# TheoBald200814/RGB-D-Instance-Segmentation

Measured on AMD Instinct MI355X. Metric: NYUv2 640x480 RGB-D img/s (fwd+bwd) of the DGGM+E-DSAM hot path, higher is better.
Workload: dtype bf16

## Files before the change

### rgb-d-instance-segmentation_amd/csrc/ratio_common.hpp

```cpp
#pragma once
#include <algorithm>

#include "mfma.hpp"
#include "timing.hpp"

namespace rgbd::rp {

constexpr int STEM_K = 160, STEM_C = 192, FUS_C = 128, ATT_C = 64, C5 = 256, C6 = 512;
constexpr int STEM_K2 = 168;
constexpr int NBN = 6;
constexpr float BN_EPS = 1e-5f;

struct Layout {
  size_t w1, b1, w2, b2, w3, b3, w4, b4, w5, b5, w6, b6, w7, b7, w8, b8, w9, b9, w10, b10;
  size_t zero;
  size_t w5q;
  size_t w1s;
  size_t w1f, w2f;
  size_t total;
};

inline Layout make_layout(int es) {
  Layout L;
  size_t o = 0;
  auto seg = [&](size_t bytes) {
    size_t r = o;
    o += align256(bytes);
    return r;
  };
  L.w1 = seg((size_t)STEM_C * STEM_K * es);
  L.b1 = seg(STEM_C * 4);
  L.w2 = seg((size_t)FUS_C * STEM_C * es);
  L.b2 = seg(FUS_C * 4);
  L.w3 = seg((size_t)ATT_C * FUS_C * es);
  L.b3 = seg(ATT_C * 4);
  L.w4 = seg((size_t)FUS_C * ATT_C * es);
  L.b4 = seg(FUS_C * 4);
  L.w5 = seg((size_t)C5 * 9 * FUS_C * es);
  L.b5 = seg(C5 * 4);
  L.w6 = seg((size_t)C6 * C5 * 9 * 4);
  L.b6 = seg(C6 * 4);
  L.w7 = seg(128 * 512 * 4);
  L.b7 = seg(128 * 4);
  L.w8 = seg(64 * 128 * 4);
  L.b8 = seg(64 * 4);
  L.w9 = seg(32 * 64 * 4);
  L.b9 = seg(32 * 4);
  L.w10 = seg(32 * 4);
  L.b10 = seg(4);
  L.zero = seg(256);
  L.w1s = seg(es == 2 ? (size_t)STEM_C * STEM_K2 * 2 : 0);
  L.w1f = seg(es == 2 ? (size_t)STEM_C * STEM_K2 * 4 : 0);
  L.w2f = seg(es == 2 ? (size_t)FUS_C * STEM_C * 4 : 0);
  L.w5q = seg(es == 2 ? (size_t)C5 * 9 * FUS_C * 2 : 0);
  L.total = o;
  return L;
}

__host__ __device__ __forceinline__ int chain_perm(int g, int e) { return e < 4 ? 4 * g + e : 16 + 4 * g + (e - 4); }

struct WPtrs {
  const float* p[RGBD_RATIO_NW];
};
struct BnPtrs {
  float* p[NBN * 4];
};

constexpr int CH_TW = 16, CH_TH = 4;
constexpr int C2W_TH = 8, C2W_TW = 32, C2W_PH = C2W_TH + 6, C2W_PW = C2W_TW + 6;
constexpr int C2W_S1 = STEM_K2 + 8, C2W_S2 = STEM_C + 8, C2W_S3 = FUS_C + 8, C2W_S4 = ATT_C + 8;
constexpr int CV_TH = 4, CV_TW = 32;
constexpr int C4_TH = 16, C4_TW = 32, C4_PW = C4_TW + 2;
constexpr int POOL_SPLIT = 16;
constexpr size_t FOLD_W1 = 0, FOLD_W2 = FOLD_W1 + (size_t)STEM_C * STEM_K2 * 2;
constexpr size_t FOLD_B1 = FOLD_W2 + (size_t)FUS_C * STEM_C * 2, FOLD_B2 = FOLD_B1 + STEM_C * 4;
constexpr size_t FOLD_BYTES = FOLD_B2 + FUS_C * 4;
inline bool stem_moments_ok(int H, int W) { return H >= 8 && W >= 8; }

__host__ __device__ __forceinline__ int c4_ph(int H) { return (H + 15) / 16 * 16 + 2; }
__host__ __device__ __forceinline__ int c4_pw(int W) { return (W + 31) / 32 * 32 + 2; }
__host__ __device__ __forceinline__ long long c4_att_idx(int b, int q, int y, int x, int H, int W) {
  return (((long long)b * 4 + q) * c4_ph(H) + y + 1) * c4_pw(W) * 32 + (long long)(x + 1) * 32;
}

struct TileDec {
  int b, y0, x0;
};
__device__ __forceinline__ TileDec tile_dec(unsigned t, unsigned per, unsigned tiles_x, int th, int tw) {
  const unsigned b = t / per, rem = t - b * per, ty = rem / tiles_x;
  return TileDec{(int)b, (int)ty * th, (int)(rem - ty * tiles_x) * tw};
}

__device__ __forceinline__ float sigmoid_fast(float x) {
  return __builtin_amdgcn_rcpf(1.f + __builtin_amdgcn_exp2f(-1.4426950408889634f * x));
}

struct BnVals {
  float g, b, rm, rv;
};
__device__ __forceinline__ BnVals bn_vals(const float* gamma, const float* beta, const float* run_mean,
                                          const float* run_var, int c) {
  return BnVals{gamma[c], beta[c], run_mean[c], run_var[c]};
}
__device__ __forceinline__ float2 bn_finish_v(double s, double q, double count, int training, float momentum,
                                              const BnVals& p, float* run_mean, float* run_var, int c,
                                              float2* __restrict__ affine) {
  float mean, var;
  if (training) {
    const double m = s / count;
    double v = q / count - m * m;
    if (v < 0.0) v = 0.0;
    mean = (float)m;
    var = (float)v;
    const double unb = count > 1.0 ? v * count / (count - 1.0) : v;
    run_mean[c] = (1.f - momentum) * p.rm + momentum * mean;
    run_var[c] = (1.f - momentum) * p.rv + momentum * (float)unb;
  } else {
    mean = p.rm;
    var = p.rv;
  }
  const float sc = p.g / sqrtf(var + BN_EPS);
  const float2 af = make_float2(sc, p.b - mean * sc);
  affine[c] = af;
  return af;
}
__device__ __forceinline__ float2 bn_finish(double s, double q, double count, int training, float momentum,
                                            const float* gamma, const float* beta, float* run_mean, float* run_var,
                                            int c, float2* __restrict__ affine) {
  return bn_finish_v(s, q, count, training, momentum, bn_vals(gamma, beta, run_mean, run_var, c), run_mean, run_var,
                     c, affine);
}
__device__ __forceinline__ void bn_affine_body(const float* __restrict__ slab, int nslab, int row, int c_off, int c,
                                               double count, int training, float momentum, const float* gamma,
                                               const float* beta, float* run_mean, float* run_var,
                                               float2* __restrict__ affine, int cm = 0) {
  __shared__ double red[2][4];
  BnVals pv{};
  if (threadIdx.x == 0) pv = bn_vals(gamma, beta, run_mean, run_var, c);
  double s = 0.0, q = 0.0;
  if (training) {
    int i = threadIdx.x;
    for (; i + 256 * 7 < nslab; i += 256 * 8) {
      float2 v[8];
#pragma unroll
      for (int u = 0; u < 8; ++u)
        v[u] = *reinterpret_cast<const float2*>(
            slab + (cm ? (long long)(c_off + c) * nslab + i + 256 * u : (long long)(i + 256 * u) * row + c_off + c) * 2);
#pragma unroll
      for (int u = 0; u < 8; ++u) {
        s += (double)v[u].x;
        q += (double)v[u].y;
      }
    }
    for (; i < nslab; i += 256) {
      const long long e = cm ? (long long)(c_off + c) * nslab + i : (long long)i * row + c_off + c;
      s += (double)slab[e * 2 + 0];
      q += (double)slab[e * 2 + 1];
    }
  }
  s = wave_sum_f64(s);
  q = wave_sum_f64(q);
  if ((threadIdx.x & 63) == 0) {
    red[0][threadIdx.x >> 6] = s;
    red[1][threadIdx.x >> 6] = q;
  }
  __syncthreads();
  if (threadIdx.x != 0) return;
  bn_finish_v(((red[0][0] + red[0][1]) + red[0][2]) + red[0][3], ((red[1][0] + red[1][1]) + red[1][2]) + red[1][3],
              count, training, momentum, pv, run_mean, run_var, c, affine);
}

__device__ inline void c4_pad_body(bf16_t* __restrict__ att, int H, int W, int bx, int plane, int nbx) {
  const int PH = c4_ph(H), PW = c4_pw(W);
  bf16_t* pl = att + (long long)plane * PH * PW * 32;
  const int edge_rows = PH - H, side = PW - W;
  const long long full = (long long)edge_rows * PW * 4, part = (long long)H * side * 4;
  for (long long i = bx * 256 + threadIdx.x; i < full + part; i += 256LL * nbx) {
    long long px;
    if (i < full) {
      const long long c = i >> 2;
      const int rr = (int)(c / PW), cc = (int)(c % PW);
      px = (long long)(rr == 0 ? 0 : H + rr) * PW + cc;
    } else {
      const long long c = (i - full) >> 2;
      const int rr = (int)(c / side), k = (int)(c % side);
      px = (long long)(rr + 1) * PW + (k == 0 ? 0 : W + k);
    }
    *reinterpret_cast<uint4*>(pl + px * 32 + 8 * (i & 3)) = make_uint4(0u, 0u, 0u, 0u);
  }
}

inline int device_cus() {
  static int n = [] {
    int dev = 0, v = 0;
    if (hipGetDevice(&dev) != hipSuccess || hipDeviceGetAttribute(&v, hipDeviceAttributeMultiprocessorCount, dev) != hipSuccess)
      v = 256;
    return v > 0 ? v : 256;
  }();
  return n;
}


int bn_affine(const float* slab, int nslab, int C, double count, int training, float momentum, const BnPtrs& bn,
              int layer, float2* affine, int cm, hipStream_t s);
int bn_affine_stem(const float* slab, int nslab, double count, int training, float momentum, const BnPtrs& bn,
                   float2* aff1, hipStream_t s);
size_t stem_ws_size(int B, int H, int W);
int stem_bn_moments(const float* depth3, long long bstride, int B, int H, int W, const char* blob, const Layout& L,
                    float momentum, const BnPtrs& bn, float2* aff1, char* fold, bf16_t* att, char* ws, hipStream_t s);

int chain_grid_v2(int B, int H, int W, int phase = 1);
int fold_bn(const char* blob, const Layout& L, const float2* aff, int which, char* fold, hipStream_t s);
int chain_v2(int phase, const float* depth3, long long bstride, int B, int H, int W, const char* blob, const Layout& L,
             const float2* aff1, const float2* aff2, const char* fold, float* slab, bf16_t* att, hipStream_t s);

int gate(const bf16_t* fus, int B, int H, int W, const char* blob, const Layout& L, const float2* aff2, bf16_t* att,
         hipStream_t s);
int c4_pad_zero(bf16_t* att, int B, int H, int W, hipStream_t s);
long long conv4_tiles(int B, int H, int W);
int conv4_grid(int B, int H, int W);
bool conv4_pool_fused(int H, int W);
int conv5_v4(int mode, const bf16_t* att, int B, int H, int W, const char* blob, const Layout& L, const float2* aff5,
             bf16_t* y, float* out, hipStream_t s);
int pool_v4(const bf16_t* y, int B, int H, int W, const float2* aff5, float* part, hipStream_t s);
int pool_finish_v4(const float* ip, int B, int H, int W, float* pooled, hipStream_t s);

int chain_grid(int B, int H, int W);
int conv_grid(int B, int H, int W);
int chain_f32(int phase, const float* depth3, long long bstride, int B, int H, int W, const char* blob,
              const Layout& L, const float2* aff1, const float2* aff2, float* slab, float* att, hipStream_t s);
int conv3x3_f32(const float* att, int B, int H, int W, const char* blob, const Layout& L, float* y, float* slab,
                hipStream_t s);
int bn_relu_pool_f32(const float* y, int B, int H, int W, const float2* aff5, float* part, hipStream_t s);

int pool_finish(const float* part, int B, int H, int W, float* pooled, hipStream_t s);
int tail(const float* pooled, int B, int training, float momentum, const char* blob, const Layout& L,
         const BnPtrs& bn, unsigned long long seed, unsigned long long* seed_ctr, float* feat, float* h1, float* ratio,
         hipStream_t s);

}
```

### rgb-d-instance-segmentation_amd/csrc/ratio_conv5.hip

```cpp
#include "ratio_common.hpp"

using namespace rgbd;
using namespace rgbd::rp;

namespace {

constexpr int GT_S = FUS_C + 8;
constexpr size_t GT_OFF_W3 = 0;
constexpr size_t GT_OFF_W4 = GT_OFF_W3 + (size_t)ATT_C * C2W_S3 * 2;
constexpr size_t GT_OFF_B = GT_OFF_W4 + (size_t)FUS_C * C2W_S4 * 2;
constexpr size_t GT_OFF_IMG = GT_OFF_B + (size_t)(ATT_C + FUS_C + 2 * FUS_C) * 4;
constexpr size_t GT_SMEM = GT_OFF_IMG + (size_t)8 * C2W_TW * GT_S * 2;
static_assert(GT_SMEM <= 163840, "gate LDS budget");

__global__ __launch_bounds__(512) void k_rp_gate(const bf16_t* __restrict__ fus, int B, int H, int W,
                                                 const char* __restrict__ blob, Layout L,
                                                 const float2* __restrict__ aff2, bf16_t* __restrict__ att) {
  extern __shared__ __attribute__((aligned(16))) char smem[];
  const bf16_t* sW3 = (const bf16_t*)(smem + GT_OFF_W3);
  const bf16_t* sW4 = (const bf16_t*)(smem + GT_OFF_W4);
  float* sb3 = (float*)(smem + GT_OFF_B);
  float* sb4 = sb3 + ATT_C;
  float2* saff = (float2*)(sb4 + FUS_C);
  const int tid = threadIdx.x, lane = tid & 63, wave = tid >> 6;
  const int r = lane & 15, g = lane >> 4;
  bf16_t* img = (bf16_t*)(smem + GT_OFF_IMG) + (size_t)wave * C2W_TW * GT_S;
  {
    auto copy_rows = [&](size_t dst, size_t src, int rows, int k, int stride) {
      const int per = k / 8;
      for (int i = tid; i < rows * per; i += 512) {
        const int rr = i / per, q = i % per;
        *reinterpret_cast<uint4*>(smem + dst + ((size_t)rr * stride + 8 * q) * 2) =
            *reinterpret_cast<const uint4*>(blob + src + ((size_t)rr * k + 8 * q) * 2);
      }
    };
    copy_rows(GT_OFF_W3, L.w3, ATT_C, FUS_C, C2W_S3);
    copy_rows(GT_OFF_W4, L.w4, FUS_C, ATT_C, C2W_S4);
    for (int i = tid; i < ATT_C; i += 512) sb3[i] = ((const float*)(blob + L.b3))[i];
    for (int i = tid; i < FUS_C; i += 512) {
      sb4[i] = ((const float*)(blob + L.b4))[i];
      saff[i] = aff2[i];
    }
  }
  __syncthreads();
  const int tiles_x = (W + C2W_TW - 1) / C2W_TW, tiles_y = (H + C2W_TH - 1) / C2W_TH;
  const unsigned per = (unsigned)(tiles_x * tiles_y);
  const int ntiles = B * tiles_x * tiles_y;
  uint2 nxt[8][2];
  auto fetch = [&](int tl) {
    if (tl >= ntiles) return;
    const int tp = ntiles - 1 - tl;
    const bf16_t* ft = fus + (((long long)tp * 8 + wave) * 16) * 256;
#pragma unroll
    for (int t = 0; t < 8; ++t) {
      const u32x4 q = __builtin_nontemporal_load(reinterpret_cast<const u32x4*>(ft + (t * 64 + lane) * 8));
      nxt[t][0] = make_uint2(q[0], q[1]);
      nxt[t][1] = make_uint2(q[2], q[3]);
    }
  };
  fetch(blockIdx.x);
  for (int tile = blockIdx.x; tile < ntiles; tile += gridDim.x) {
    const TileDec td = tile_dec((unsigned)(ntiles - 1 - tile), per, (unsigned)tiles_x, C2W_TH, C2W_TW);
    const int b = td.b, y0 = td.y0, x0 = td.x0;
    const int py = y0 + wave;
    uint2 raw[8][2];
#pragma unroll
    for (int t = 0; t < 8; ++t)
#pragma unroll
      for (int u = 0; u < 2; ++u) raw[t][u] = nxt[t][u];
    fetch(tile + gridDim.x);
    if (py >= H) continue;
    asm volatile("s_waitcnt lgkmcnt(0)" ::: "memory");
#pragma unroll
    for (int t = 0; t < 8; ++t) {
      const int c = 16 * t + r;
      const float2 a = saff[c];
#pragma unroll
      for (int u = 0; u < 2; ++u) {
        const uint32_t w01 = raw[t][u].x, w23 = raw[t][u].y;
        const float v[4] = {__uint_as_float(w01 << 16), __uint_as_float(w01 & 0xffff0000u),
                            __uint_as_float(w23 << 16), __uint_as_float(w23 & 0xffff0000u)};
#pragma unroll
        for (int j = 0; j < 4; ++j)
          img[(16 * u + 4 * g + j) * GT_S + c] = f32_to_bf16(fmaxf(__builtin_fmaf(v[j], a.x, a.y), 0.f));
      }
    }
    __builtin_amdgcn_wave_barrier();
    asm volatile("s_waitcnt lgkmcnt(0)" ::: "memory");
    Frag<bf16_t> f2[4][2];
#pragma unroll
    for (int s = 0; s < 4; ++s)
#pragma unroll
      for (int u = 0; u < 2; ++u) {
        const bf16_t* row = img + (16 * u + r) * GT_S + 32 * s + 4 * g;
        const uint2 lo = *reinterpret_cast<const uint2*>(row), hi = *reinterpret_cast<const uint2*>(row + 16);
        f2[s][u].v = make_uint4(lo.x, lo.y, hi.x, hi.y);
      }
    f32x4 a3[4][2];
#pragma unroll
    for (int t = 0; t < 4; ++t) {
      const float4 bb = *reinterpret_cast<const float4*>(sb3 + 16 * t + 4 * g);
      a3[t][0] = a3[t][1] = f32x4{bb.x, bb.y, bb.z, bb.w};
#pragma unroll
      for (int s = 0; s < 4; ++s) {
        Frag<bf16_t> af;
        af.v = *reinterpret_cast<const uint4*>(sW3 + (16 * t + r) * C2W_S3 + 32 * s + 8 * g);
        mma(a3[t][0], af, f2[s][0]);
        mma(a3[t][1], af, f2[s][1]);
      }
    }
    Frag<bf16_t> f3[2][2];
#pragma unroll
    for (int s = 0; s < 2; ++s)
#pragma unroll
      for (int u = 0; u < 2; ++u) {
        float vv[8];
#pragma unroll
        for (int e = 0; e < 8; ++e) vv[e] = fmaxf(a3[2 * s + (e >> 2)][u][e & 3], 0.f);
        f3[s][u].from8(vv);
      }
#pragma unroll
    for (int t = 0; t < 8; ++t) {
      const float4 bb = *reinterpret_cast<const float4*>(sb4 + 16 * t + 4 * g);
      f32x4 a4[2] = {f32x4{bb.x, bb.y, bb.z, bb.w}, f32x4{bb.x, bb.y, bb.z, bb.w}};
#pragma unroll
      for (int s = 0; s < 2; ++s) {
        Frag<bf16_t> af;
        af.v = *reinterpret_cast<const uint4*>(sW4 + (16 * t + r) * C2W_S4 + 32 * s + 8 * g);
        mma(a4[0], af, f3[s][0]);
        mma(a4[1], af, f3[s][1]);
      }
#pragma unroll
      for (int u = 0; u < 2; ++u) {
        uint2* cell = reinterpret_cast<uint2*>(img + (16 * u + r) * GT_S + 16 * t + 4 * g);
        const uint2 act = *cell;
        const float av[4] = {__uint_as_float(act.x << 16), __uint_as_float(act.x & 0xffff0000u),
                             __uint_as_float(act.y << 16), __uint_as_float(act.y & 0xffff0000u)};
        float o[4];
#pragma unroll
        for (int j = 0; j < 4; ++j) o[j] = av[j] * sigmoid_fast(a4[u][j]);
        *cell = make_uint2(pack_bf16x2(o[0], o[1]), pack_bf16x2(o[2], o[3]));
      }
    }
    __builtin_amdgcn_wave_barrier();
    asm volatile("s_waitcnt lgkmcnt(0)" ::: "memory");
#pragma unroll
    for (int k = 0; k < 8; ++k) {
      const int qt = k >> 1, pr = 16 * (k & 1) + (lane >> 2), q = lane & 3;
      if (x0 + pr < W)
        *reinterpret_cast<uint4*>(att + c4_att_idx(b, qt, py, x0 + pr, H, W) + 8 * q) =
            *reinterpret_cast<const uint4*>(img + pr * GT_S + 32 * qt + 8 * q);
    }
  }
}

constexpr int C4_NPIX = (C4_TH + 2) * C4_PW;
constexpr int C4_APIECES = 39;
constexpr int C4_A_BYTES = C4_APIECES * 1024;
constexpr int C4_STEPS = 12;
constexpr int C4_B_BYTES = 3 * 128 * 64;
constexpr int C4_B_OFF = 2 * C4_A_BYTES;
constexpr int C4_RED_OFF = C4_B_OFF + 2 * C4_B_BYTES;
constexpr int C4_RED_BYTES = 8 * 4 * 128 * 4;
constexpr int C4_PAR_OFF = C4_RED_OFF + C4_RED_BYTES;
constexpr size_t C4_SMEM = C4_PAR_OFF + 128 * 4 + 128 * 8 + 32 * 4;
static_assert(C4_SMEM <= 163840, "conv5 v4 LDS budget");
static_assert(C4_APIECES * 16 >= C4_NPIX && C4_APIECES % 3 == 0, "conv5 v4 input pieces");
constexpr int C4_AK = (C4_APIECES + 3) / 4;
static_assert(2 * C4_A_BYTES >= 8 * 128 * 2 * 4, "conv5 v4 statistics scratch");

__device__ __forceinline__ uint32_t c4_off(int row, int chunk) { return row * 64 + 16 * (chunk ^ ((row >> 1) & 2)); }

struct C4Tile {
  int b, y0, x0;
};
__device__ __forceinline__ C4Tile c4_tile(long long t, int tiles_x, int tiles_y) {
  C4Tile o;
  const long long per = (long long)tiles_x * tiles_y;
  o.b = (int)(t / per);
  const int rem = (int)(t % per);
  o.y0 = (rem / tiles_x) * C4_TH;
  o.x0 = (rem % tiles_x) * C4_TW;
  return o;
}

#ifndef C4_NODMA
#define C4_NODMA 0
#endif


#if defined(RGBD_DIAG) && !defined(C4_STAMPS)
#define C4_STAMPS
#endif
#ifdef C4_STAMPS
__device__ unsigned long long* g_c4_stamps = nullptr;
__device__ __forceinline__ void c4_stamp(unsigned long long* st, long long idx) {
  __builtin_amdgcn_sched_barrier(0);
  const unsigned long long t = __builtin_amdgcn_s_memtime();
  if ((threadIdx.x & 63) == 0) st[idx] = t;
  __builtin_amdgcn_sched_barrier(0);
}
#define C4_STAMP(k) \
  if (sts) c4_stamp(sts, (((long long)tcount * C4_STEPS + st) * 8 + wave) * 5 + (k))
#else
#define C4_STAMP(k)
#endif
template <int MODE>
__global__ __launch_bounds__(512) void k_rp_conv5_v4(const bf16_t* __restrict__ x, int B, int H, int W,
                                                     const char* __restrict__ blob, Layout L,
                                                     const float2* __restrict__ aff, bf16_t* __restrict__ y,
                                                     float* __restrict__ out, int xcd_pairs) {
  extern __shared__ __attribute__((aligned(1024))) char smem[];
  const int tid = threadIdx.x, lane = tid & 63;
  const int wave = __builtin_amdgcn_readfirstlane(tid >> 6);
  const int r = lane & 15, g = lane >> 4;
  const uint32_t lds0 = (uint32_t)(uintptr_t)smem;
  int pair, nh;
  if (xcd_pairs) {
    nh = (blockIdx.x >> 3) & 1;
    pair = (blockIdx.x & 7) | ((blockIdx.x >> 4) << 3);
  } else {
    nh = blockIdx.x & 1;
    pair = blockIdx.x >> 1;
  }
  const int npairs = gridDim.x >> 1;
  const char* w5q = blob + L.w5q + (size_t)nh * C4_STEPS * C4_B_BYTES;
  float* sbias = (float*)(smem + C4_PAR_OFF);
  float2* saff = (float2*)(smem + C4_PAR_OFF + 512);
  int* sslot = (int*)(smem + C4_PAR_OFF + 512 + 1024);
  for (int i = tid; i < 128; i += 512) {
    sbias[i] = ((const float*)(blob + L.b5))[nh * 128 + i];
    if constexpr (MODE == 1) saff[i] = aff[nh * 128 + i];
  }
  const int tiles_x = (W + C4_TW - 1) / C4_TW, tiles_y = (H + C4_TH - 1) / C4_TH;
  const long long ntiles = (long long)B * tiles_x * tiles_y;

  const int PW = c4_pw(W);
  const long long plane = (long long)c4_ph(H) * PW * 32;
  uint32_t aoff[C4_AK];
#pragma unroll
  for (int k = 0; k < C4_AK; ++k) {
    const int row = 16 * ((wave & 3) + 4 * k) + (lane >> 2), q = lane & 3;
    const int hy = row / C4_PW, hx = row - hy * C4_PW;
    aoff[k] = row < C4_NPIX ? (uint32_t)((hy * PW + hx) * 64 + 16 * (q ^ ((row >> 1) & 2))) : 0u;
  }
  auto issue_a = [&](const C4Tile& t, int qt, int sl, int k) {
    const char* base = (const char*)(x + ((long long)t.b * 4 + qt) * plane + ((long long)t.y0 * PW + t.x0) * 32);
    dma_lds16(base + aoff[k], lds0 + sl * C4_A_BYTES + ((wave & 3) + 4 * k) * 1024);
  };
  auto issue_b = [&](int st, int k0, int k1) {
    const char* src = w5q + (size_t)st * C4_B_BYTES + 16 * lane;
    const uint32_t dst = lds0 + C4_B_OFF + (st & 1) * C4_B_BYTES;
    for (int k = k0; k < k1; ++k) dma_lds16(src + 1024 * k, dst + 1024 * k);
  };
  const bool loader = wave < 4;

  f32x2 ssum[8], ssq[8];
#pragma unroll
  for (int nj = 0; nj < 8; ++nj) ssum[nj] = ssq[nj] = f32x2{0.f, 0.f};
  const int rh = H >> 2, rw = W >> 2;

#ifndef C4_NOPRIO
  if (wave >= 4) __builtin_amdgcn_s_setprio(1);
#endif
  long long tile = pair;
  if (tile < ntiles) {
    const C4Tile t = c4_tile(tile, tiles_x, tiles_y);
    if (!loader) {
#pragma unroll
      for (int k = 0; k < C4_AK; ++k)
        if ((wave & 3) + 4 * k < C4_APIECES) issue_a(t, 0, 0, k);
    }
    issue_b(0, 3 * wave, 3 * wave + 3);
  }
  asm volatile("s_waitcnt vmcnt(0)" ::: "memory");
  __syncthreads();

#ifdef C4_STAMPS
  int tcount = 0;
#endif
  for (; tile < ntiles; tile += npairs) {
#ifdef C4_STAMPS
    unsigned long long* const sts = (blockIdx.x == 0 && tcount < 2) ? g_c4_stamps : nullptr;
#endif
    const C4Tile t = c4_tile(tile, tiles_x, tiles_y);
    const long long ntile = tile + npairs;
    const bool has_next = ntile < ntiles;
    const C4Tile tn = c4_tile(has_next ? ntile : tile, tiles_x, tiles_y);
    f32x4 acc[4][8];
#pragma unroll
    for (int mi = 0; mi < 4; ++mi)
#pragma unroll
      for (int nj = 0; nj < 8; ++nj) acc[mi][nj] = f32x4{0.f, 0.f, 0.f, 0.f};

#pragma unroll 1
    for (int st = 0; st < C4_STEPS; ++st) {
      const int qt = st / 3, ky = st - 3 * qt;
      C4_STAMP(0);
      if (!(C4_NODMA & 1) && loader && (st + 1 < C4_STEPS || has_next))
        issue_b(st + 1 < C4_STEPS ? st + 1 : 0, 6 * wave, 6 * wave + 6);
      C4_STAMP(1);
      const int qn = qt + 1;
      const bool a_go = !(C4_NODMA & 2) && !loader && (qn < 4 || has_next);
      const char* sa = smem + (qt & 1) * C4_A_BYTES;
      const char* sb = smem + C4_B_OFF + (st & 1) * C4_B_BYTES;
#pragma unroll
      for (int kx = 0; kx < 3; ++kx) {
        Frag<bf16_t> fa[4], fb[8];
        if constexpr (!(C4_NODMA & 8)) {
#pragma unroll
          for (int mi = 0; mi < 4; ++mi) {
            const int p = (2 * wave + (mi >> 1) + ky) * C4_PW + (mi & 1) * 16 + r + kx;
            fa[mi].v = *reinterpret_cast<const uint4*>(sa + c4_off(p, g));
          }
#pragma unroll
          for (int nj = 0; nj < 8; ++nj) fb[nj].v = *reinterpret_cast<const uint4*>(sb + c4_off(kx * 128 + 16 * nj + r, g));
        } else {
#pragma unroll
          for (int mi = 0; mi < 4; ++mi) fa[mi].v = make_uint4(lane, kx, st, mi);
#pragma unroll
          for (int nj = 0; nj < 8; ++nj) fb[nj].v = make_uint4(nj, lane, kx, st);
        }
#pragma unroll
        for (int mi = 0; mi < 4; ++mi)
#pragma unroll
          for (int nj = 0; nj < 8; ++nj) mma(acc[mi][nj], fa[mi], fb[nj]);
        if (kx == 0 && a_go) {
#pragma unroll
          for (int k = 0; k < C4_AK; ++k) {
            const int j = (wave & 3) + 4 * k;
            if (j >= 13 * ky && j < 13 * ky + 13 && j < C4_APIECES) issue_a(qn < 4 ? t : tn, qn & 3, qn & 1, k);
          }
        }
        if (kx == 0) C4_STAMP(2);
      }
      C4_STAMP(3);
      if constexpr (C4_NODMA & 4)
        asm volatile("s_waitcnt vmcnt(0) lgkmcnt(0)" ::: "memory");
      else
        asm volatile("s_waitcnt vmcnt(0) lgkmcnt(0)\n\ts_barrier" ::: "memory");
      C4_STAMP(4);
    }
#ifdef C4_STAMPS
    ++tcount;
#endif

    const long long item = 2 * tile + nh;
    if constexpr (MODE != 1) {
      bf16_t* yt = y + ((item * 8 + wave) * 16) * 512;
      const bool interior = t.y0 + C4_TH <= H && t.x0 + C4_TW <= W;
#pragma unroll
      for (int np = 0; np < 4; ++np) {
        const float b0 = sbias[32 * np + r], b1 = sbias[32 * np + 16 + r];
        if (interior) {
          const f32x2 bb0 = {b0, b0}, bb1 = {b1, b1};
#pragma unroll
          for (int mi = 0; mi < 4; ++mi) {
            const f32x4 v = acc[mi][2 * np], w = acc[mi][2 * np + 1];
            const f32x2 a0 = f32x2{v[0], v[1]} + bb0, a1 = f32x2{v[2], v[3]} + bb0;
            const f32x2 c0 = f32x2{w[0], w[1]} + bb1, c1 = f32x2{w[2], w[3]} + bb1;
            const u32x4 pk = {pack_bf16x2(a0.x, a0.y), pack_bf16x2(a1.x, a1.y), pack_bf16x2(c0.x, c0.y),
                              pack_bf16x2(c1.x, c1.y)};
            __builtin_nontemporal_store(pk, reinterpret_cast<u32x4*>(yt + ((mi * 4 + np) * 64 + lane) * 8));
            if constexpr (MODE == 0) {
              ssum[2 * np] += a0 + a1;
              ssq[2 * np] = __builtin_elementwise_fma(a0, a0, __builtin_elementwise_fma(a1, a1, ssq[2 * np]));
              ssum[2 * np + 1] += c0 + c1;
              ssq[2 * np + 1] = __builtin_elementwise_fma(c0, c0, __builtin_elementwise_fma(c1, c1, ssq[2 * np + 1]));
            }
          }
        } else {
#pragma unroll
          for (int mi = 0; mi < 4; ++mi) {
            const bool row_ok = t.y0 + 2 * wave + (mi >> 1) < H;
            const int xb = t.x0 + (mi & 1) * 16 + 4 * g;
            uint32_t hv[8];
#pragma unroll
            for (int h = 0; h < 2; ++h) {
              const int nj = 2 * np + h;
              const float bias = h ? b1 : b0;
#pragma unroll
              for (int j = 0; j < 4; ++j) {
                const float av = acc[mi][nj][j] + bias;
                hv[4 * h + j] = (uint32_t)f32_to_bf16(av);
                if (MODE == 0 && row_ok && xb + j < W) {
                  ssum[nj].x += av;
                  ssq[nj].x = __builtin_fmaf(av, av, ssq[nj].x);
                }
              }
            }
            *reinterpret_cast<uint4*>(yt + ((mi * 4 + np) * 64 + lane) * 8) =
                make_uint4(hv[0] | (hv[1] << 16), hv[2] | (hv[3] << 16), hv[4] | (hv[5] << 16), hv[6] | (hv[7] << 16));
          }
        }
      }
    } else {
      float* red = (float*)(smem + C4_RED_OFF);
      if (tid < 32) {
        const int row = t.y0 + 2 * (tid >> 2) + ((tid & 3) >> 1), col = t.x0 + 16 * (tid & 1);
        sslot[tid] = row < H ? (row / rh - t.y0 / rh) * 2 + (col / rw - t.x0 / rw) : -1;
      }
#pragma unroll
      for (int mi = 0; mi < 4; ++mi)
#pragma unroll
        for (int nj = 0; nj < 8; ++nj) {
          const float bias = sbias[16 * nj + r];
          const float2 a = saff[16 * nj + r];
          float s = 0.f;
#pragma unroll
          for (int j = 0; j < 4; ++j) {
            const float vb = bf16_to_f32(f32_to_bf16(acc[mi][nj][j] + bias));
            s += fmaxf(vb * a.x + a.y, 0.f);
          }
          s += __shfl_xor(s, 16);
          s += __shfl_xor(s, 32);
          if (g == 0) red[(wave * 4 + mi) * 128 + 16 * nj + r] = s;
        }
      __syncthreads();
      {
        const int slot = tid >> 7, c = tid & 127;
        float s = 0.f;
        for (int f = 0; f < 32; ++f)
          if (sslot[f] == slot) s += red[f * 128 + c];
        out[(item * 4 + slot) * 128 + c] = s;
      }
    }
  }
  if constexpr (MODE == 0) {
    asm volatile("s_waitcnt vmcnt(0)" ::: "memory");
    __syncthreads();
    float* red = (float*)smem;
#pragma unroll
    for (int nj = 0; nj < 8; ++nj) {
      float a = ssum[nj].x + ssum[nj].y, q = ssq[nj].x + ssq[nj].y;
      a += __shfl_xor(a, 16);
      a += __shfl_xor(a, 32);
      q += __shfl_xor(q, 16);
      q += __shfl_xor(q, 32);
      if (g == 0) {
        red[(wave * 128 + 16 * nj + r) * 2] = a;
        red[(wave * 128 + 16 * nj + r) * 2 + 1] = q;
      }
    }
    __syncthreads();
    for (int i = tid; i < C5 * 2; i += 512) {
      const int c = i >> 1, k = i & 1;
      float v = 0.f;
      if ((c >> 7) == nh)
        for (int w = 0; w < 8; ++w) v += red[(w * 128 + (c & 127)) * 2 + k];
      out[((long long)c * gridDim.x + blockIdx.x) * 2 + k] = v;
    }
  }
}

__global__ __launch_bounds__(256) void k_rp_bn_relu_pool_v4_tiles(const bf16_t* __restrict__ y, int H, int W,
                                                                  const float2* __restrict__ aff,
                                                                  float* __restrict__ part) {
  __shared__ float red[C5];
  const int b = (int)gridDim.y - 1 - (int)blockIdx.y;
  const int reg = blockIdx.x / POOL_SPLIT, sp = blockIdx.x % POOL_SPLIT;
  const int i = reg / 4, j = reg % 4;
  const int tiles_x = W / C4_TW, tiles_y = H / C4_TH;
  const int rhy = H / 32, rtx = W / 128;
  const int t = threadIdx.x, lane = t & 63, np = t >> 6, r = lane & 15;
  float2 af[2][2];
#pragma unroll
  for (int nh = 0; nh < 2; ++nh)
#pragma unroll
    for (int h = 0; h < 2; ++h) af[nh][h] = aff[nh * 128 + 32 * np + 16 * h + r];
  float acc[2][2] = {{0.f, 0.f}, {0.f, 0.f}};
  for (int q = sp; q < rhy * rtx; q += POOL_SPLIT) {
    const int hy = i * rhy + q / rtx, tx = j * rtx + q % rtx;
    const long long tile = ((long long)b * tiles_y + (hy >> 1)) * tiles_x + tx;
#pragma unroll
    for (int nh = 0; nh < 2; ++nh) {
      const uint4* src = reinterpret_cast<const uint4*>(y + ((2 * tile + nh) * 8 + 4 * (hy & 1)) * 16 * 512) + t;
      uint4 v[16];
#pragma unroll
      for (int u = 0; u < 16; ++u) {
        const u32x4 xv = __builtin_nontemporal_load(reinterpret_cast<const u32x4*>(src + 256 * u));
        v[u] = make_uint4(xv.x, xv.y, xv.z, xv.w);
      }
#pragma unroll
      for (int u = 0; u < 16; ++u) {
        const uint32_t w[4] = {v[u].x, v[u].y, v[u].z, v[u].w};
#pragma unroll
        for (int h = 0; h < 2; ++h)
#pragma unroll
          for (int e = 0; e < 2; ++e) {
            const float lo = __uint_as_float(w[2 * h + e] << 16), hi = __uint_as_float(w[2 * h + e] & 0xffff0000u);
            acc[nh][h] += fmaxf(lo * af[nh][h].x + af[nh][h].y, 0.f);
            acc[nh][h] += fmaxf(hi * af[nh][h].x + af[nh][h].y, 0.f);
          }
      }
    }
  }
#pragma unroll
  for (int nh = 0; nh < 2; ++nh)
#pragma unroll
    for (int h = 0; h < 2; ++h) {
      float v = acc[nh][h];
      v += __shfl_xor(v, 16);
      v += __shfl_xor(v, 32);
      if (lane < 16) red[nh * 128 + 32 * np + 16 * h + r] = v;
    }
  __syncthreads();
  part[(((long long)b * 16 + reg) * POOL_SPLIT + sp) * C5 + t] = red[t];
}

__global__ __launch_bounds__(256) void k_rp_bn_relu_pool_v4_frag(const bf16_t* __restrict__ y, int H, int W,
                                                                 const float2* __restrict__ aff,
                                                                 float* __restrict__ part) {
  __shared__ float red[2][C5];
  const int b = blockIdx.y, reg = blockIdx.x / POOL_SPLIT, sp = blockIdx.x % POOL_SPLIT;
  const int i = reg / 4, j = reg % 4;
  const int cp = threadIdx.x & 127, ql = threadIdx.x >> 7;
  const int nh = cp >> 6, np = (cp >> 4) & 3, r = cp & 15, n0 = nh * 128 + 32 * np + r, n1 = n0 + 16;
  const int ya = (i * H) / 4, yb = ((i + 1) * H + 3) / 4, xa = (j * W) / 4, xb = ((j + 1) * W + 3) / 4;
  const int rows = yb - ya;
  const int r0 = ya + (rows * sp) / POOL_SPLIT, r1 = ya + (rows * (sp + 1)) / POOL_SPLIT;
  const int qa = xa >> 2, nq = ((xb + 3) >> 2) - qa;
  const int tiles_x = (W + C4_TW - 1) / C4_TW, tiles_y = (H + C4_TH - 1) / C4_TH;
  const float2 a0 = aff[n0], a1 = aff[n1];
  float s0 = 0.f, s1 = 0.f;
  constexpr int PU = 8;
  int yy = r0, k = ql;
  while (k >= nq) {
    k -= nq;
    ++yy;
  }
  while (yy < r1) {
    uint4 v[PU];
    int xqs[PU];
    bool ok[PU];
#pragma unroll
    for (int u = 0; u < PU; ++u) {
      ok[u] = yy < r1;
      const int ry = ok[u] ? yy : r1 - 1, xq = (qa + (ok[u] ? k : 0)) * 4;
      xqs[u] = xq;
      const long long tile = ((long long)b * tiles_y + ry / C4_TH) * tiles_x + xq / C4_TW;
      const int ly = ry % C4_TH, lx = xq % C4_TW;
      const int wave = ly >> 1, mi = (ly & 1) * 2 + (lx >> 4), g = (lx & 15) >> 2;
      v[u] = *reinterpret_cast<const uint4*>(y + (((((2 * tile + nh) * 8 + wave) * 4 + mi) * 4 + np) * 64 + g * 16 + r) * 8);
      k += 2;
      while (k >= nq) {
        k -= nq;
        ++yy;
      }
    }
#pragma unroll
    for (int u = 0; u < PU; ++u) {
      const uint32_t w0[4] = {v[u].x, v[u].y, v[u].z, v[u].w};
#pragma unroll
      for (int e = 0; e < 4; ++e) {
        const int xx = xqs[u] + e;
        if (ok[u] && xx >= xa && xx < xb) {
          const float c0 = bf16_to_f32((bf16_t)(e & 1 ? w0[e >> 1] >> 16 : w0[e >> 1] & 0xffff));
          const float c1 = bf16_to_f32((bf16_t)(e & 1 ? w0[2 + (e >> 1)] >> 16 : w0[2 + (e >> 1)] & 0xffff));
          s0 += fmaxf(c0 * a0.x + a0.y, 0.f);
          s1 += fmaxf(c1 * a1.x + a1.y, 0.f);
        }
      }
    }
  }
  red[ql][n0] = s0;
  red[ql][n1] = s1;
  __syncthreads();
  const int c = threadIdx.x;
  part[(((long long)b * 16 + reg) * POOL_SPLIT + sp) * C5 + c] = red[0][c] + red[1][c];
}

__global__ __launch_bounds__(256) void k_rp_pool_finish_v4(const float* __restrict__ ip, int B, int H, int W,
                                                           float* __restrict__ pooled) {
  const int b = blockIdx.y, reg = blockIdx.x, i = reg / 4, j = reg % 4, c = threadIdx.x;
  const int nh = c >> 7, cc = c & 127;
  const int rh = H >> 2, rw = W >> 2;
  const int tiles_x = W / C4_TW, tiles_y = (H + C4_TH - 1) / C4_TH;
  const int ty0 = (i * rh) / C4_TH, ty1 = ((i + 1) * rh - 1) / C4_TH;
  const int tx0 = (j * rw) / C4_TW, tx1 = ((j + 1) * rw - 1) / C4_TW;
  float s = 0.f;
  for (int ty = ty0; ty <= ty1; ++ty)
    for (int tx = tx0; tx <= tx1; ++tx) {
      const int slot = (i - (ty * C4_TH) / rh) * 2 + (j - (tx * C4_TW) / rw);
      const long long tile = ((long long)b * tiles_y + ty) * tiles_x + tx;
      s += ip[((2 * tile + nh) * 4 + slot) * 128 + cc];
    }
  pooled[((long long)b * C5 + c) * 16 + reg] = s / (float)(rh * rw);
}

__global__ __launch_bounds__(256) void k_c4_pad_zero(bf16_t* __restrict__ att, int H, int W) {
  c4_pad_body(att, H, W, blockIdx.x, blockIdx.y, gridDim.x);
}

inline int gate_grid(int B, int H, int W) {
  return (int)std::min<long long>((long long)B * ((W + 31) / 32) * ((H + 7) / 8), device_cus());
}

template <int MODE>
int conv5_launch(const bf16_t* att, int B, int H, int W, const char* blob, const Layout& L, const float2* aff5,
                 bf16_t* y, float* out, hipStream_t s) {
  static const hipError_t sattr = hipFuncSetAttribute((const void*)k_rp_conv5_v4<MODE>,
                                                      hipFuncAttributeMaxDynamicSharedMemorySize, (int)C4_SMEM);
  if (sattr != hipSuccess) return (int)sattr;
  const int gcv = conv4_grid(B, H, W);
  k_rp_conv5_v4<MODE><<<gcv, 512, C4_SMEM, s>>>(att, B, H, W, blob, L, aff5, y, out, gcv % 16 == 0);
  return RGBD_OK;
}

}

namespace rgbd::rp {

int gate(const bf16_t* fus, int B, int H, int W, const char* blob, const Layout& L, const float2* aff2, bf16_t* att,
         hipStream_t s) {
  TimerScope ts("rp_chain", s);
  static const hipError_t gattr =
      hipFuncSetAttribute((const void*)k_rp_gate, hipFuncAttributeMaxDynamicSharedMemorySize, (int)GT_SMEM);
  if (gattr != hipSuccess) return (int)gattr;
  k_rp_gate<<<gate_grid(B, H, W), 512, GT_SMEM, s>>>(fus, B, H, W, blob, L, aff2, att);
  return RGBD_OK;
}

int c4_pad_zero(bf16_t* att, int B, int H, int W, hipStream_t s) {
  k_c4_pad_zero<<<dim3(8, B * 4), 256, 0, s>>>(att, H, W);
  return RGBD_OK;
}

long long conv4_tiles(int B, int H, int W) {
  return (long long)B * ((W + C4_TW - 1) / C4_TW) * ((H + C4_TH - 1) / C4_TH);
}
int conv4_grid(int B, int H, int W) { return 2 * (int)std::min<long long>(conv4_tiles(B, H, W), device_cus() / 2); }
bool conv4_pool_fused(int H, int W) { return H % 4 == 0 && W % 64 == 0 && H >= 64 && W >= 128; }

int conv5_v4(int mode, const bf16_t* att, int B, int H, int W, const char* blob, const Layout& L, const float2* aff5,
             bf16_t* y, float* out, hipStream_t s) {
  TimerScope ts("rp_conv3x3", s);
  return mode == 0   ? conv5_launch<0>(att, B, H, W, blob, L, aff5, y, out, s)
         : mode == 1 ? conv5_launch<1>(att, B, H, W, blob, L, aff5, y, out, s)
                     : conv5_launch<2>(att, B, H, W, blob, L, aff5, y, out, s);
}

int pool_v4(const bf16_t* y, int B, int H, int W, const float2* aff5, float* part, hipStream_t s) {
  if (H % 32 == 0 && W % 128 == 0)
    k_rp_bn_relu_pool_v4_tiles<<<dim3(16 * POOL_SPLIT, B), 256, 0, s>>>(y, H, W, aff5, part);
  else
    k_rp_bn_relu_pool_v4_frag<<<dim3(16 * POOL_SPLIT, B), 256, 0, s>>>(y, H, W, aff5, part);
  return RGBD_OK;
}

int pool_finish_v4(const float* ip, int B, int H, int W, float* pooled, hipStream_t s) {
  k_rp_pool_finish_v4<<<dim3(16, B), 256, 0, s>>>(ip, B, H, W, pooled);
  return RGBD_OK;
}

}

#ifdef RGBD_DIAG
extern "C" int rgbd_debug_conv5_stamps(void* buf) {
  unsigned long long* p = (unsigned long long*)buf;
  return (int)hipMemcpyToSymbol(HIP_SYMBOL(g_c4_stamps), &p, sizeof(p));
}
#endif
```

Before: 3115.

## Use transposing LDS reads with swizzled channel-major staging in the gate kernel

After: 3153, median of 6. About the same (+1.2%).

```diff
diff --git a/rgb-d-instance-segmentation_amd/csrc/ratio_common.hpp b/rgb-d-instance-segmentation_amd/csrc/ratio_common.hpp
--- a/rgb-d-instance-segmentation_amd/csrc/ratio_common.hpp
+++ b/rgb-d-instance-segmentation_amd/csrc/ratio_common.hpp
@@ -94,6 +94,11 @@
 __device__ __forceinline__ float sigmoid_fast(float x) {
   return __builtin_amdgcn_rcpf(1.f + __builtin_amdgcn_exp2f(-1.4426950408889634f * x));
 }
+__device__ __forceinline__ f32x2 sigmoid_fast2(f32x2 x) {
+  const f32x2 m = f32x2{-1.4426950408889634f, -1.4426950408889634f} * x;
+  const f32x2 d = f32x2{1.f, 1.f} + f32x2{__builtin_amdgcn_exp2f(m.x), __builtin_amdgcn_exp2f(m.y)};
+  return f32x2{__builtin_amdgcn_rcpf(d.x), __builtin_amdgcn_rcpf(d.y)};
+}
 
 struct BnVals {
   float g, b, rm, rv;
diff --git a/rgb-d-instance-segmentation_amd/csrc/ratio_conv5.hip b/rgb-d-instance-segmentation_amd/csrc/ratio_conv5.hip
--- a/rgb-d-instance-segmentation_amd/csrc/ratio_conv5.hip
+++ b/rgb-d-instance-segmentation_amd/csrc/ratio_conv5.hip
@@ -6,12 +6,36 @@
 namespace {
 
 constexpr int GT_S = FUS_C + 8;
+static_assert(C2W_TW * GT_S * 2 >= FUS_C * C2W_TW * 2, "the [ch][px] image fits the wave's region");
+typedef short gt_v4s __attribute__((ext_vector_type(4)));
+typedef short gt_v2s __attribute__((ext_vector_type(2)));
+typedef unsigned int gt_u2 __attribute__((ext_vector_type(2)));
+typedef __attribute__((address_space(3))) char gt_lds_char;
+typedef __attribute__((address_space(3))) gt_v4s gt_lds_v4s;
+typedef __attribute__((address_space(3))) gt_u2 gt_lds_u2;
+typedef __attribute__((address_space(3))) u32x4 gt_lds_u4;
+__device__ __forceinline__ int gt_swz(int c) { return ((c >> 1) & 1) | (((c >> 3) & 1) << 1) | (((c >> 2) & 1) << 2); }
+__device__ __forceinline__ f32x2 bf16x2_to_f32x2(uint32_t w) {
+  return f32x2{__uint_as_float(w << 16), __uint_as_float(w & 0xffff0000u)};
+}
+__device__ __forceinline__ float gt_fma(float v, float sc, float sh) {
+  float d;
+  asm("v_fma_f32 %0, %1, %2, %3" : "=v"(d) : "v"(v), "v"(sc), "v"(sh));
+  return d;
+}
+__device__ __forceinline__ uint32_t relu_bf16x2(uint32_t p) {
+  return __builtin_bit_cast(uint32_t, __builtin_elementwise_max(__builtin_bit_cast(gt_v2s, p), gt_v2s{0, 0}));
+}
 constexpr size_t GT_OFF_W3 = 0;
 constexpr size_t GT_OFF_W4 = GT_OFF_W3 + (size_t)ATT_C * C2W_S3 * 2;
 constexpr size_t GT_OFF_B = GT_OFF_W4 + (size_t)FUS_C * C2W_S4 * 2;
 constexpr size_t GT_OFF_IMG = GT_OFF_B + (size_t)(ATT_C + FUS_C + 2 * FUS_C) * 4;
 constexpr size_t GT_SMEM = GT_OFF_IMG + (size_t)8 * C2W_TW * GT_S * 2;
 static_assert(GT_SMEM <= 163840, "gate LDS budget");
+
+#ifndef GT_NOMATH
+#define GT_NOMATH 0
+#endif
 
 __global__ __launch_bounds__(512) void k_rp_gate(const bf16_t* __restrict__ fus, int B, int H, int W,
                                                  const char* __restrict__ blob, Layout L,
@@ -22,9 +46,18 @@
   float* sb3 = (float*)(smem + GT_OFF_B);
   float* sb4 = sb3 + ATT_C;
   float2* saff = (float2*)(sb4 + FUS_C);
-  const int tid = threadIdx.x, lane = tid & 63, wave = tid >> 6;
+  const int tid = threadIdx.x, lane = tid & 63;
+  const int wave = __builtin_amdgcn_readfirstlane(tid >> 6);
   const int r = lane & 15, g = lane >> 4;
-  bf16_t* img = (bf16_t*)(smem + GT_OFF_IMG) + (size_t)wave * C2W_TW * GT_S;
+  gt_lds_char* const tin = (gt_lds_char*)(smem + GT_OFF_IMG) + wave * (C2W_TW * GT_S * 2);
+  int wr_off[2], rd_off[2], out_off[2];
+#pragma unroll
+  for (int u = 0; u < 2; ++u) {
+    const int row = 4 * g + (r >> 2);
+    wr_off[u] = 64 * r + 8 * ((4 * u + g) ^ gt_swz(r));
+    rd_off[u] = 64 * row + 8 * ((4 * u + (r & 3)) ^ gt_swz(row));
+    out_off[u] = ((16 * u + r) * GT_S + 4 * g) * 2;
+  }
   {
     auto copy_rows = [&](size_t dst, size_t src, int rows, int k, int stride) {
       const int per = k / 8;
@@ -70,32 +103,34 @@
       for (int u = 0; u < 2; ++u) raw[t][u] = nxt[t][u];
     fetch(tile + gridDim.x);
     if (py >= H) continue;
-    asm volatile("s_waitcnt lgkmcnt(0)" ::: "memory");
+    asm volatile("" ::: "memory");
 #pragma unroll
     for (int t = 0; t < 8; ++t) {
-      const int c = 16 * t + r;
-      const float2 a = saff[c];
+      const float2 a = saff[16 * t + r];
 #pragma unroll
       for (int u = 0; u < 2; ++u) {
-        const uint32_t w01 = raw[t][u].x, w23 = raw[t][u].y;
-        const float v[4] = {__uint_as_float(w01 << 16), __uint_as_float(w01 & 0xffff0000u),
-                            __uint_as_float(w23 << 16), __uint_as_float(w23 & 0xffff0000u)};
-#pragma unroll
-        for (int j = 0; j < 4; ++j)
-          img[(16 * u + 4 * g + j) * GT_S + c] = f32_to_bf16(fmaxf(__builtin_fmaf(v[j], a.x, a.y), 0.f));
-      }
-    }
-    __builtin_amdgcn_wave_barrier();
-    asm volatile("s_waitcnt lgkmcnt(0)" ::: "memory");
+        if constexpr (GT_NOMATH) {
+          *reinterpret_cast<gt_lds_u2*>(tin + wr_off[u] + 1024 * t) = gt_u2{raw[t][u].x, raw[t][u].y};
+          continue;
+        }
+        const f32x2 v01 = bf16x2_to_f32x2(raw[t][u].x), v23 = bf16x2_to_f32x2(raw[t][u].y);
+        *reinterpret_cast<gt_lds_u2*>(tin + wr_off[u] + 1024 * t) =
+            gt_u2{relu_bf16x2(pack_bf16x2(gt_fma(v01.x, a.x, a.y), gt_fma(v01.y, a.x, a.y))),
+                  relu_bf16x2(pack_bf16x2(gt_fma(v23.x, a.x, a.y), gt_fma(v23.y, a.x, a.y)))};
+      }
+    }
+    asm volatile("" ::: "memory");
     Frag<bf16_t> f2[4][2];
 #pragma unroll
     for (int s = 0; s < 4; ++s)
 #pragma unroll
       for (int u = 0; u < 2; ++u) {
-        const bf16_t* row = img + (16 * u + r) * GT_S + 32 * s + 4 * g;
-        const uint2 lo = *reinterpret_cast<const uint2*>(row), hi = *reinterpret_cast<const uint2*>(row + 16);
-        f2[s][u].v = make_uint4(lo.x, lo.y, hi.x, hi.y);
-      }
+        const gt_v4s lo = __builtin_amdgcn_ds_read_tr16_b64_v4i16((gt_lds_v4s*)(tin + rd_off[u] + 2048 * s));
+        const gt_v4s hi = __builtin_amdgcn_ds_read_tr16_b64_v4i16((gt_lds_v4s*)(tin + rd_off[u] + 2048 * s + 1024));
+        const gt_u2 l2 = __builtin_bit_cast(gt_u2, lo), h2 = __builtin_bit_cast(gt_u2, hi);
+        f2[s][u].v = make_uint4(l2.x, l2.y, h2.x, h2.y);
+      }
+    asm volatile("" ::: "memory");
     f32x4 a3[4][2];
 #pragma unroll
     for (int t = 0; t < 4; ++t) {
@@ -114,10 +149,9 @@
     for (int s = 0; s < 2; ++s)
 #pragma unroll
       for (int u = 0; u < 2; ++u) {
-        float vv[8];
-#pragma unroll
-        for (int e = 0; e < 8; ++e) vv[e] = fmaxf(a3[2 * s + (e >> 2)][u][e & 3], 0.f);
-        f3[s][u].from8(vv);
+        const f32x4 lo = a3[2 * s][u], hi = a3[2 * s + 1][u];
+        f3[s][u].v = make_uint4(relu_bf16x2(pack_bf16x2(lo[0], lo[1])), relu_bf16x2(pack_bf16x2(lo[2], lo[3])),
+                                relu_bf16x2(pack_bf16x2(hi[0], hi[1])), relu_bf16x2(pack_bf16x2(hi[2], hi[3])));
       }
 #pragma unroll
     for (int t = 0; t < 8; ++t) {
@@ -132,24 +166,23 @@
       }
 #pragma unroll
       for (int u = 0; u < 2; ++u) {
-        uint2* cell = reinterpret_cast<uint2*>(img + (16 * u + r) * GT_S + 16 * t + 4 * g);
-        const uint2 act = *cell;
-        const float av[4] = {__uint_as_float(act.x << 16), __uint_as_float(act.x & 0xffff0000u),
-                             __uint_as_float(act.y << 16), __uint_as_float(act.y & 0xffff0000u)};
-        float o[4];
-#pragma unroll
-        for (int j = 0; j < 4; ++j) o[j] = av[j] * sigmoid_fast(a4[u][j]);
-        *cell = make_uint2(pack_bf16x2(o[0], o[1]), pack_bf16x2(o[2], o[3]));
-      }
-    }
-    __builtin_amdgcn_wave_barrier();
-    asm volatile("s_waitcnt lgkmcnt(0)" ::: "memory");
+        const uint4 fv = f2[t >> 1][u].v;
+        if constexpr (GT_NOMATH) {
+          *reinterpret_cast<gt_lds_u2*>(tin + out_off[u] + 32 * t) = t & 1 ? gt_u2{fv.z, fv.w} : gt_u2{fv.x, fv.y};
+          continue;
+        }
+        const f32x2 o01 = bf16x2_to_f32x2(t & 1 ? fv.z : fv.x) * sigmoid_fast2(f32x2{a4[u][0], a4[u][1]});
+        const f32x2 o23 = bf16x2_to_f32x2(t & 1 ? fv.w : fv.y) * sigmoid_fast2(f32x2{a4[u][2], a4[u][3]});
+        *reinterpret_cast<gt_lds_u2*>(tin + out_off[u] + 32 * t) =
+            gt_u2{pack_bf16x2(o01.x, o01.y), pack_bf16x2(o23.x, o23.y)};
+      }
+    }
+    asm volatile("" ::: "memory");
 #pragma unroll
     for (int k = 0; k < 8; ++k) {
       const int qt = k >> 1, pr = 16 * (k & 1) + (lane >> 2), q = lane & 3;
-      if (x0 + pr < W)
-        *reinterpret_cast<uint4*>(att + c4_att_idx(b, qt, py, x0 + pr, H, W) + 8 * q) =
-            *reinterpret_cast<const uint4*>(img + pr * GT_S + 32 * qt + 8 * q);
+      const u32x4 ov = *reinterpret_cast<const gt_lds_u4*>(tin + (pr * GT_S + 32 * qt + 8 * q) * 2);
+      if (x0 + pr < W) *reinterpret_cast<u32x4*>(att + c4_att_idx(b, qt, py, x0 + pr, H, W) + 8 * q) = ov;
     }
   }
 }
```
